# JackShDr/InfluentialRS

Measured on AMD Instinct MI355X. Metric: scored user-item pairs/sec (whole node), higher is better.
Workload: dtype f32; 1 GPU; c2: n_item=3415, d=128, L=200, H=4, layers=6, ffn=256; one greedy path-search step; users_per_gpu=4096, top_k=100, sweep=bf16 filter + exact f32 re-score, parallelism=single GPU

## Files before the change

influentialrs_amd/csrc/decoder.hip:

```cpp
#include "irs_internal.h"

typedef __attribute__((ext_vector_type(16))) float f32x16;

__global__ void __launch_bounds__(256) k_embed(const int64_t *__restrict__ seq, const float *__restrict__ E,
                                               const float *__restrict__ pe, float *__restrict__ x, int rows, int L,
                                               int d, float sqrtd, int64_t n_item) {
    int row = blockIdx.x * 4 + (threadIdx.x >> 6);
    int lane = threadIdx.x & 63;
    if (row >= rows) return;
    int64_t id = seq[row];
    if (id < 0) id = 0;
    if (id > n_item) id = n_item;
    int t = row % L;
    const float *e = E + id * (int64_t)d;
    const float *p = pe + (int64_t)t * d;
    float *o = x + (int64_t)row * d;
    for (int c = lane; c < d; c += 64) o[c] = __fadd_rn(__fmul_rn(e[c], sqrtd), p[c]);
}

__global__ void k_pif(const int64_t *__restrict__ user, const float *__restrict__ U, const float *__restrict__ w,
                      const float *__restrict__ b, float *__restrict__ r_u, int B, int ud, int64_t n_user) {
    int i = blockIdx.x * blockDim.x + threadIdx.x;
    if (i >= B) return;
    int64_t u = user[i];
    if (u < 0) u = 0;
    if (u >= n_user) u = n_user - 1;
    const float *e = U + u * (int64_t)ud;
    float acc = 0.f;
    for (int c = 0; c < ud; ++c) acc = __fmaf_rn(e[c], w[c], acc);
    r_u[i] = acc + b[0];
}

__global__ void k_fill(float *p, float v, int n) {
    int i = blockIdx.x * blockDim.x + threadIdx.x;
    if (i < n) p[i] = v;
}

__global__ void k_cross_const(const float *__restrict__ Wo, const float *__restrict__ b_in, const float *__restrict__ bo,
                              float *__restrict__ c, int d) {
    int i = blockIdx.x * blockDim.x + threadIdx.x;
    if (i >= d) return;
    const float *bv = b_in + 2 * d;
    float acc = 0.f;
    for (int j = 0; j < d; ++j) acc = __fmaf_rn(Wo[(int64_t)i * d + j], bv[j], acc);
    c[i] = acc + bo[i];
}

__device__ __forceinline__ bool plan_valid(const int64_t *__restrict__ sq, int t, int L, int p) {
    return t < L && (sq[t] != 0 || t == p);
}

__global__ void __launch_bounds__(256) k_plan_count(const int64_t *__restrict__ seq, const int32_t *__restrict__ pos, int B,
                                                    int L, int32_t *__restrict__ cnt, int32_t *__restrict__ tile_seq) {
    const int b = blockIdx.x * 4 + (threadIdx.x >> 6), lane = threadIdx.x & 63;
    if (b >= B) return;
    if (tile_seq && lane < 16) tile_seq[16 * b + lane] = -1;
    int p = pos[b];
    p = p < 0 ? 0 : (p >= L ? L - 1 : p);
    const int64_t *sq = seq + (int64_t)b * L;
    int n = 0;
    for (int t0 = 0; t0 < L; t0 += 64) n += __popcll(__ballot(plan_valid(sq, t0 + lane, L, p)));
    if (lane == 0) cnt[b] = n;
}

__global__ void __launch_bounds__(1024) k_plan_scan(const int32_t *__restrict__ cnt, int B, int32_t *__restrict__ off,
                                                    int32_t *__restrict__ m_dev) {
    __shared__ int s_scan[1024];
    __shared__ int s_base;
    const int tid = threadIdx.x;
    if (tid == 0) s_base = 0;
    __syncthreads();
    for (int b0 = 0; b0 < B; b0 += 1024) {
        const int b = b0 + tid;
        const int n = (b < B) ? cnt[b] : 0;
        s_scan[tid] = n;
        __syncthreads();
        for (int o = 1; o < 1024; o <<= 1) {
            int v = (tid >= o) ? s_scan[tid - o] : 0;
            __syncthreads();
            s_scan[tid] += v;
            __syncthreads();
        }
        const int base = s_base;
        if (b < B) off[b] = base + s_scan[tid] - n;
        __syncthreads();
        if (tid == 1023) s_base = base + s_scan[1023];
        __syncthreads();
    }
    if (tid == 0) m_dev[0] = s_base;
}

__global__ void __launch_bounds__(256) k_plan_fill(const int64_t *__restrict__ seq, const int32_t *__restrict__ pos, int B,
                                                   int L, const int32_t *__restrict__ off, int32_t *__restrict__ qrow,
                                                   int32_t *__restrict__ tok_row, int32_t *__restrict__ padq) {
    const int b = blockIdx.x * 4 + (threadIdx.x >> 6), lane = threadIdx.x & 63;
    if (b >= B) return;
    int p = pos[b];
    p = p < 0 ? 0 : (p >= L ? L - 1 : p);
    const int64_t *sq = seq + (int64_t)b * L;
    int o = off[b];
    for (int t0 = 0; t0 < L; t0 += 64) {
        const int t = t0 + lane;
        const bool v = plan_valid(sq, t, L, p);
        const unsigned long long m = __ballot(v);
        if (v) {
            const int idx = o + __popcll(m & ((1ull << lane) - 1ull));
            tok_row[idx] = b * L + t;
            if (t == p) {
                qrow[b] = idx;
                padq[b] = (sq[t] == 0) ? idx - off[b] : -1;
            }
        }
        o += __popcll(m);
    }
}

static int irs_cu_count() {
    static int n_cu = 0;
    if (n_cu == 0) {
        int dev = 0;
        if (hipGetDevice(&dev) != hipSuccess ||
            hipDeviceGetAttribute(&n_cu, hipDeviceAttributeMultiprocessorCount, dev) != hipSuccess || n_cu <= 0)
            n_cu = 256;
    }
    return n_cu;
}

#define SEQ_WG_TILES 8
#define SEQ_WG_BLOCKS 16
#define SEQ_AUTO_MIN_SEQS 384
#define SEQ_RMAX 48
#define SEQ_TAIL_BLOCKS 8
#ifndef SEQ_LAB_PLAN
#define SEQ_LAB_PLAN 0
#endif
__host__ __device__ __forceinline__ int seq_half_of_block(bool slot_odd, int nb, int blk) {
    const int mir = nb - 1 - blk;
    if (!slot_odd) {
        if ((nb & 1) && blk == mir) return nb - 1;
        return blk < mir ? 2 * blk : 2 * mir + 1;
    }
    if (nb & 1) {
        if (blk == mir) return 0;
        return blk < mir ? 1 + 2 * blk : 2 + 2 * mir;
    }
    if (blk == nb / 2 - 1) return 0;
    if (blk == nb / 2) return nb - 1;
    return blk < mir ? 1 + 2 * blk : 2 + 2 * mir;
}
#define SEQ_PLAN_PER_THREAD 8
__global__ void __launch_bounds__(1024) k_plan_seq(const int32_t *__restrict__ cnt, const int32_t *__restrict__ off,
                                                   const int32_t *__restrict__ qrow, int B, int32_t *__restrict__ tile_seq,
                                                   int32_t *__restrict__ tile_qb, int32_t *__restrict__ seq_row0,
                                                   int32_t *__restrict__ qrow_tile, int32_t *__restrict__ n_wg, int tiles_cap,
                                                   int n_cu) {
    constexpr int C = SEQ_WG_BLOCKS, PT = SEQ_PLAN_PER_THREAD, CT = SEQ_TAIL_BLOCKS;
    __shared__ int s_hist[C + 1], s_start[C + 2];
    __shared__ int p_n[C], p_s[C][SEQ_RMAX], p_l[C][SEQ_RMAX];
    __shared__ int c_cum[C + 1], c_q[C], c_exist, c_newbase, s_nwg;
    __shared__ int s_cap, s_tail0, c_norm, c_nnorm;
    __shared__ unsigned short s_order[1024 * PT], s_pt[1024 * PT];
    const int tid = threadIdx.x;
    if (tid <= C) s_hist[tid] = 0;
    if (tid < C) p_n[tid] = 0;
    if (tid == 0) s_nwg = 0, s_tail0 = -1;
    __syncthreads();
    int my_T[PT], my_rk[PT];
#pragma unroll
    for (int j = 0; j < PT; ++j) {
        const int b = tid + 1024 * j;
        my_T[j] = 0, my_rk[j] = 0;
        if (b < B) {
            int nb = (cnt[b] + 15) >> 4;
            nb = nb < 1 ? 1 : (nb > C ? C : nb);
            my_T[j] = nb;
            int pt = qrow[b] - off[b];
            s_pt[b] = (unsigned short)(pt < 0 ? 0 : (pt > 65535 ? 65535 : pt));
        }
    }
#pragma unroll
    for (int j = 0; j < PT; ++j)
        if (my_T[j]) my_rk[j] = atomicAdd(&s_hist[my_T[j]], 1);
    __syncthreads();
    if (tid == 0) {
        int run = 0;
        for (int T = C; T >= 1; --T) {
            s_start[T] = run;
            run += s_hist[T];
        }
        auto count = [&](const int cap, int &nwg, int &nbig, int &ntail) __attribute__((always_inline)) {
            int dc[C];
            nwg = 0, nbig = 0, ntail = 0;
#pragma unroll
            for (int f = 0; f < C; ++f) dc[f] = 0;
#pragma unroll
            for (int T = C; T >= 1; --T) {
                int left = s_hist[T];
                if (left > 0) {
#pragma unroll
                    for (int f = T; f < C; ++f) {
                        const int q = f / T, have = dc[f] * q, used = left < have ? left : have;
                        if (used > 0) {
                            const int fl = used / q, pa = used - fl * q;
                            left -= used;
                            dc[f] -= fl + (pa ? 1 : 0), dc[f - T * q] += fl;
#pragma unroll
                            for (int p = 1; p < q; ++p)
                                if (pa == p) dc[f - T * p] += 1;
                        }
                    }
                    const int q = C / T;
                    if (T <= CT) {
                        const int qt = T <= CT ? CT / T : 1, room = cap > nwg ? cap - nwg : 0;
                        if ((long long)room * q < left) {
                            const int tl = left - room * q, flt = tl / qt, pat = tl - flt * qt;
                            left = room * q;
                            dc[CT - T * qt] += flt, nwg += flt + (pat ? 1 : 0), ntail += flt + (pat ? 1 : 0);
#pragma unroll
                            for (int p = 1; p < qt; ++p)
                                if (pat == p) dc[CT - T * p] += 1;
                        }
                    }
                    const int fl = left / q, pa = left - fl * q;
                    dc[C - T * q] += fl, nwg += fl + (pa ? 1 : 0);
#pragma unroll
                    for (int p = 1; p < q; ++p)
                        if (pa == p) dc[C - T * p] += 1;
                }
                if (T == CT + 1) nbig = nwg;
            }
        };
        int nwg, nbig, ntail;
        count(0x7FFFFFFF, nwg, nbig, ntail);
        const int rounds = n_cu > 0 ? nwg / n_cu : 0, rem = nwg - rounds * n_cu;
        s_cap = 0x7FFFFFFF;
        if (SEQ_LAB_PLAN == 0 && n_cu > 0 && rem > 0 && 2 * rem <= n_cu && nbig <= rounds * n_cu) {
            int nwg2, nbig2;
            count(rounds * n_cu, nwg2, nbig2, ntail);
            if (ntail <= n_cu) s_cap = rounds * n_cu;
        }
        if (SEQ_LAB_PLAN == 1) s_cap = 0;
        if (SEQ_LAB_PLAN == 2) s_cap = 0x7FFFFFFF;
    }
    __syncthreads();
#pragma unroll
    for (int j = 0; j < PT; ++j)
        if (my_T[j]) s_order[s_start[my_T[j]] + my_rk[j]] = (unsigned short)(tid + 1024 * j);
    __syncthreads();
    auto pool_bins = [&](int f) {
        int n = 0;
        for (int r = 0; r < p_n[f]; ++r) n += p_l[f][r];
        return n;
    };
    auto append = [&](int f, int start, int len) {
        if (f < 1 || len < 1) return;
        if (p_n[f] > 0 && p_s[f][p_n[f] - 1] + p_l[f][p_n[f] - 1] == start) p_l[f][p_n[f] - 1] += len;
        else if (p_n[f] < SEQ_RMAX) p_s[f][p_n[f]] = start, p_l[f][p_n[f]] = len, ++p_n[f];
    };
    auto take_prefix = [&](int f, int m, int dest) {
        for (int r = 0; r < p_n[f] && m > 0; ++r) {
            const int t = m < p_l[f][r] ? m : p_l[f][r];
            append(dest, p_s[f][r], t);
            p_s[f][r] += t, p_l[f][r] -= t, m -= t;
        }
        int w = 0;
        for (int r = 0; r < p_n[f]; ++r)
            if (p_l[f][r] > 0) p_s[f][w] = p_s[f][r], p_l[f][w] = p_l[f][r], ++w;
        p_n[f] = w;
    };
    for (int T = C; T >= 1; --T) {
        const int n = s_hist[T], qnew = C / T;
        if (n == 0) continue;
        if (tid == 0) {
            int tot = 0;
            for (int f = T; f < C; ++f) {
                c_cum[f] = tot, c_q[f] = f / T;
                tot += pool_bins(f) * c_q[f];
            }
            c_cum[C] = tot;
            c_exist = n < tot ? n : tot;
            c_newbase = s_nwg;
            const int nnew = n - c_exist, room = s_cap > s_nwg ? s_cap - s_nwg : 0;
            const bool spill = T <= CT && nnew > 0 && (long long)room * qnew < nnew;
            c_norm = spill ? room * qnew : nnew;
            c_nnorm = (c_norm + qnew - 1) / qnew;
            const int ntail = spill ? (nnew - c_norm + CT / T - 1) / (CT / T) : 0;
            if (ntail > 0 && s_tail0 < 0) s_tail0 = c_newbase + c_nnorm;
            s_nwg += c_nnorm + ntail;
        }
        __syncthreads();
        const int exist = c_exist, base = s_start[T];
        for (int i = tid; i < n; i += 1024) {
            const int b = s_order[base + i];
            int w, slot;
            if (i < exist) {
                int f = T;
                while (f < C - 1 && i >= c_cum[f + 1]) ++f;
                const int s_ = i - c_cum[f];
                int bl = s_ / c_q[f];
                const int k = s_ % c_q[f];
                int r = 0;
                while (r < p_n[f] - 1 && bl >= p_l[f][r]) bl -= p_l[f][r], ++r;
                w = p_s[f][r] + bl;
                slot = (C - f) + k * T;
            } else if (i - exist < c_norm) {
                const int j_ = i - exist;
                w = c_newbase + j_ / qnew;
                slot = (j_ % qnew) * T;
            } else {
                const int j_ = i - exist - c_norm, qt = CT / T;
                w = c_newbase + c_nnorm + j_ / qt;
                slot = (C - CT) + (j_ % qt) * T;
            }
            if (w * SEQ_WG_TILES >= tiles_cap) continue;
            const int h0 = 2 * SEQ_WG_TILES * w + slot;
            for (int blk = 0; blk < T; ++blk) {
                const int h = h0 + seq_half_of_block(slot & 1, T, blk);
                tile_seq[h] = b, tile_qb[h] = blk;
            }
            seq_row0[b] = 16 * slot;
            const int pt = s_pt[b];
            int pb = pt >> 4;
            pb = pb < 0 ? 0 : (pb >= T ? T - 1 : pb);
            qrow_tile[b] = 16 * (h0 + seq_half_of_block(slot & 1, T, pb)) + (pt & 15);
        }
        __syncthreads();
        if (tid == 0) {
            int left = exist;
            for (int f = T; f < C && left > 0; ++f) {
                const int q = c_q[f], cap = pool_bins(f) * q;
                const int used = left < cap ? left : cap;
                left -= used;
                const int full = used / q, part = used % q;
                take_prefix(f, full, f - T * q);
                if (part) take_prefix(f, 1, f - T * part);
            }
            const int nnew = c_norm, fullnew = nnew / qnew, partnew = nnew % qnew;
            append(C - T * qnew, c_newbase, fullnew);
            if (partnew) append(C - T * partnew, c_newbase + fullnew, 1);
            if (n - exist > c_norm) {
                const int ntl = n - exist - c_norm, qt = CT / T, fullt = ntl / qt, partt = ntl % qt;
                append(CT - T * qt, c_newbase + c_nnorm, fullt);
                if (partt) append(CT - T * partt, c_newbase + c_nnorm + fullt, 1);
            }
        }
        __syncthreads();
    }
    if (tid == 0) n_wg[0] = s_nwg, n_wg[1] = s_tail0 < 0 ? s_nwg : s_tail0;
}

__global__ void __launch_bounds__(1024) k_plan_small(const int64_t *__restrict__ seq, const int32_t *__restrict__ pos, int B, int L,
                                                     int32_t *__restrict__ cnt, int32_t *__restrict__ off,
                                                     int32_t *__restrict__ qrow, int32_t *__restrict__ tok_row,
                                                     int32_t *__restrict__ padq, int32_t *__restrict__ m_dev,
                                                     const int64_t *__restrict__ user, const float *__restrict__ U,
                                                     const float *__restrict__ uw, const float *__restrict__ ub,
                                                     float *__restrict__ r_u, int ud, int64_t n_user,
                                                     int32_t *__restrict__ step_pair) {
    __shared__ int s_cnt[64], s_off[64];
    const int tid = threadIdx.x, wave = tid >> 6, lane = tid & 63;
    for (int b = wave; b < B; b += 16) {
        int p = pos[b];
        p = p < 0 ? 0 : (p >= L ? L - 1 : p);
        const int64_t *sq = seq + (int64_t)b * L;
        int n = 0;
        for (int t0 = 0; t0 < L; t0 += 64) n += __popcll(__ballot(plan_valid(sq, t0 + lane, L, p)));
        if (lane == 0) s_cnt[b] = n;
    }
    if (tid < B) {
        float acc = 0.f;
        if (U) {
            int64_t u = user[tid];
            if (u < 0) u = 0;
            if (u >= n_user) u = n_user - 1;
            const float *e = U + u * (int64_t)ud;
            for (int c = 0; c < ud; ++c) acc = __fmaf_rn(e[c], uw[c], acc);
            acc += ub[0];
        }
        r_u[tid] = acc;
    }
    __syncthreads();
    if (tid == 0) {
        int run = 0;
        for (int b = 0; b < B; ++b) {
            s_off[b] = run;
            run += s_cnt[b];
        }
        m_dev[0] = run;
        if (step_pair) step_pair[0] = step_pair[1];
    }
    __syncthreads();
    for (int b = wave; b < B; b += 16) {
        int p = pos[b];
        p = p < 0 ? 0 : (p >= L ? L - 1 : p);
        const int64_t *sq = seq + (int64_t)b * L;
        int o = s_off[b];
        if (lane == 0) {
            cnt[b] = s_cnt[b];
            off[b] = o;
        }
        const int o0 = o;
        for (int t0 = 0; t0 < L; t0 += 64) {
            const int t = t0 + lane;
            const bool v = plan_valid(sq, t, L, p);
            const unsigned long long m = __ballot(v);
            if (v) {
                const int idx = o + __popcll(m & ((1ull << lane) - 1ull));
                tok_row[idx] = b * L + t;
                if (t == p) {
                    qrow[b] = idx;
                    padq[b] = (sq[t] == 0) ? idx - o0 : -1;
                }
            }
            o += __popcll(m);
        }
    }
}

__global__ void __launch_bounds__(256) k_embed_packed(const int64_t *__restrict__ seq, const float *__restrict__ E,
                                                      const float *__restrict__ pe, float *__restrict__ x,
                                                      const int32_t *__restrict__ tok_row, const int32_t *__restrict__ m_dev,
                                                      int L, int d, float sqrtd, int64_t n_item) {
    const int row = blockIdx.x * 4 + (threadIdx.x >> 6);
    const int lane = threadIdx.x & 63;
    if (row >= m_dev[0]) return;
    const int orig = tok_row[row];
    int64_t id = seq[orig];
    if (id < 0) id = 0;
    if (id > n_item) id = n_item;
    const float *e = E + id * (int64_t)d;
    const float *p = pe + (int64_t)(orig % L) * d;
// ... 5358 lines not shown
    case DecFam::FRAG_FUSED:
        return frag_layer(c, l);
    case DecFam::SMALL16:
    case DecFam::WIDE:
    case DecFam::ANY: {
        SmallBlockArgs sb = small_args(ctx, r.layer, l, ctx->act_ao, x, nullptr, y, qkv_buf(c, l + 1), c.rows, c.m_dev,
                                       l + 1 < ctx->dims.n_layers);
        if (r.att_fused) {
            sb.QKVin = qkv_buf(c, l), sb.r_u = ctx->act_ru, sb.seq_last = c.seq + (ctx->dims.max_len - 1), sb.cnt = c.cnt;
            sb.padq = ctx->seq_padq, sb.mask_mode = ctx->dims.mask_mode;
        }
        launch_small(ctx, r.layer, sb, r.att_fused, c.rows > SMALL_MT2_ROWS, c.s);
        c.x = y;
        c.y = x;
        return IRS_OK;
    }
    default:
        return gemm_rest(ctx, r.layer == DecFam::GEMM_LN, l, ctx->act_ao, x, r.layer == DecFam::GEMM_LN ? y : x, y, x, c.rows, c.m_dev,
                         c.s);
    }
}

static int last_layer(const DecodeCall &c, int l, const int32_t *pos, float *xrows) {
    irs_ctx *ctx = c.ctx;
    const DecodeRoute &r = c.r;
    const int L = ctx->dims.max_len, d = ctx->dims.d, H = ctx->dims.n_heads, B = c.B;
    const irs_layer_w &w = ctx->layer[l];
    const int32_t *qrow = c.qrow;
    const hipStream_t s = c.s;
    int rc;
    float *xf = ctx->act_xf, *h_r = ctx->act_h;
    float *ao_r = ctx->act_ao, *x_r = ao_r + (size_t)B * d, *y_r = ao_r + (size_t)2 * B * d, *z_r = ao_r + (size_t)3 * B * d;
    const float *q_r = nullptr;
    const int nt = d > 128 ? d / 32 : 4;
    if (r.seq) {
#if SEQ_LAST_ABSORB
        float *um = ctx->act_h, *cq = um + (size_t)B * 4 * d;
        hipLaunchKernelGGL(k_absorb_qu, dim3((B + ABS_SQ - 1) / ABS_SQ), dim3(256), 0, s, xf, ctx->qrow_tile, w.sa_in_w, w.sa_in_b, x_r, um,
                           cq, B);
        hipLaunchKernelGGL(k_absorb_attn, dim3(B), dim3(256), 0, s, xf, um, cq, c.seq, ctx->act_ru, L, ctx->dims.mask_mode, c.off, c.cnt,
                           qrow, ctx->seq_padq, ctx->seq_row0, ctx->qrow_tile);
        hipLaunchKernelGGL(k_absorb_out, dim3((B + ABS_SO - 1) / ABS_SO), dim3(256), 0, s, um, w.sa_in_w, w.sa_in_b, ao_r, B);
#else
        hipLaunchKernelGGL(k_gather_rows_frag, dim3(B), dim3(64), 0, s, xf, ctx->qrow_tile, x_r, d, nt);
        hipLaunchKernelGGL(k_gather_rows_frag, dim3(B), dim3(64), 0, s, ctx->act_yf, ctx->qrow_tile, ao_r, d, nt);
#endif
    } else if (r.kv_only) {
        hipLaunchKernelGGL(k_gather_rows_frag, dim3(B), dim3(64), 0, s, xf, qrow, x_r, d, nt);
        LinArgs q{};
        q.X = x_r, q.W = w.sa_in_w, q.bias = w.sa_in_b, q.Y = h_r, q.M = B, q.N = d, q.K = d;
        if ((rc = launch_linear(ctx, q, s))) return rc;
        q_r = h_r;
    }
    irs_prof_begin(ctx, IRS_PROF_ATTN, s);
    if (r.seq) {
    } else if (d / H == 32 && L <= 256 && d % 4 == 0 && (((uintptr_t)ctx->act_qkv | (uintptr_t)q_r) & 15) == 0)
        hipLaunchKernelGGL(k_attn_row32, dim3(H, B), dim3(256), 0, s, ctx->act_qkv, c.seq, ctx->act_ru, ao_r, L, d,
                           ctx->dims.mask_mode, c.off, c.cnt, qrow, q_r, ctx->seq_padq);
    else
        hipLaunchKernelGGL(k_attn_row, dim3(H, B), dim3(64), 0, s, ctx->act_qkv, c.seq, ctx->act_ru, pos, ao_r, L, d, d / H,
                           ctx->dims.mask_mode, c.off, c.cnt, c.tok, qrow, q_r);
    irs_prof_end(ctx, IRS_PROF_ATTN, s, 4.0 * B * (double)L * d, 4.0 * 3.0 * B * (double)L * d);
    const bool small = r.tail == DecFam::SMALL16 || r.tail == DecFam::WIDE || r.tail == DecFam::ANY;
    const bool idx_res = small && !r.frag;
    if (r.frag && !r.kv_only) hipLaunchKernelGGL(k_gather_rows_frag, dim3(B), dim3(64), 0, s, xf, qrow, x_r, d, nt);
    else if (!r.frag && !idx_res) hipLaunchKernelGGL(k_gather_rows_idx, dim3(B), dim3(64), 0, s, c.x, qrow, x_r, d);
    if (small) {
        const SmallBlockArgs sb = small_args(ctx, r.tail, l, ao_r, idx_res ? c.x : x_r, idx_res ? qrow : nullptr, xrows, nullptr, B,
                                             nullptr, false);
        launch_small(ctx, r.tail, sb, false, B > 2048, s);
    } else if ((rc = gemm_rest(ctx, r.tail == DecFam::GEMM_LN, l, ao_r, x_r, y_r, z_r, xrows, B, nullptr, s))) {
        return rc;
    }
    IRS_CHECK_HIP(ctx, hipGetLastError());
    return IRS_OK;
}

int irs_launch_decode(irs_ctx *ctx, const int64_t *seq, const int64_t *user, int B, float *x_out, const int32_t *pos,
                      float *xrows, float *r_u_out, hipStream_t s) {
    const int L = ctx->dims.max_len, d = ctx->dims.d, nl = ctx->dims.n_layers;
    const DecodeRoute r = decode_route(ctx, B, x_out == nullptr && pos && xrows && L >= 4);
    int rc;
    if (ctx->step_pair && !r.small_plan) IRS_FAIL(ctx, IRS_E_STATE, "merged path step needs the single-workgroup plan kernel");
    if (!r.small_plan && (rc = irs_launch_pif(ctx, user, B, ctx->act_ru, s)) != IRS_OK) return rc;
    ctx->seq_last = r.seq;
    const int32_t packed[IRS_ROUTE_FIELDS] = {r.rows_only, r.small_plan, (int32_t)r.plan, (int32_t)r.embed, (int32_t)r.layer,
                                              (int32_t)r.tail, r.frag, r.seq, r.kv_planes, r.att_fused, r.kv_only, r.x6, r.npl, r.nt};
    for (int i = 0; i < IRS_ROUTE_FIELDS; ++i) ctx->route_last[i] = packed[i];
    ctx->route_n = IRS_ROUTE_FIELDS;
    DecodeCall c{ctx, r, seq, B, B * L, ctx->act_x, ctx->act_y, s};
    if (r.rows_only) c.off = ctx->seq_off, c.cnt = ctx->seq_cnt, c.tok = ctx->tok_row, c.qrow = ctx->seq_qrow, c.m_dev = ctx->m_dev;
    if (r.plan == DecPlan::SMALL) {
        hipLaunchKernelGGL(k_plan_small, dim3(1), dim3(1024), 0, s, seq, pos, B, L, ctx->seq_cnt, ctx->seq_off, ctx->seq_qrow,
                           ctx->tok_row, ctx->seq_padq, ctx->m_dev, user, pif_table(ctx), ctx->um_w, ctx->um_b, ctx->act_ru,
                           ctx->dims.u_dim, ctx->dims.n_user, ctx->step_pair);
    } else if (r.plan == DecPlan::MULTI) {
        hipLaunchKernelGGL(k_plan_count, dim3((B + 3) / 4), dim3(256), 0, s, seq, pos, B, L, ctx->seq_cnt, ctx->tile_seq);
        hipLaunchKernelGGL(k_plan_scan, dim3(1), dim3(1024), 0, s, ctx->seq_cnt, B, ctx->seq_off, ctx->m_dev);
        hipLaunchKernelGGL(k_plan_fill, dim3((B + 3) / 4), dim3(256), 0, s, seq, pos, B, L, ctx->seq_off, ctx->seq_qrow, ctx->tok_row,
                           ctx->seq_padq);
    }
    const int n_cu = r.seq ? irs_cu_count() : 0;
    if (r.seq)
        hipLaunchKernelGGL(k_plan_seq, dim3(1), dim3(1024), 0, s, ctx->seq_cnt, ctx->seq_off, ctx->seq_qrow, B, ctx->tile_seq,
                           ctx->tile_idx, ctx->seq_row0, ctx->qrow_tile, ctx->n_wg_dev, B * SEQ_WG_TILES, n_cu);
    launch_embed(c, pos, user);
    IRS_CHECK_HIP(ctx, hipGetLastError());
    if (r_u_out) IRS_CHECK_HIP(ctx, hipMemcpyAsync(r_u_out, ctx->act_ru, sizeof(float) * B, hipMemcpyDeviceToDevice, s));
    const bool embed_qkv = r.embed == DecEmbed::SEQ || r.embed == DecEmbed::FRAG_QKV || r.embed == DecEmbed::SMALL16_QKV ||
                           r.embed == DecEmbed::ANY_QKV;
    const int l0 = r.seq ? nl - 1 : 0;
    for (int l = l0; l < nl; ++l) {
        const irs_layer_w &w = ctx->layer[l];
        if (!(l == l0 ? embed_qkv : fam_writes_qkv(r.layer))) {
            LinArgs q{};
            q.X = c.x, q.Xf = r.frag ? ctx->act_xf : nullptr, q.W = w.sa_in_w, q.bias = w.sa_in_b, q.Y = ctx->act_qkv;
            q.M = c.rows, q.N = 3 * d, q.K = d, q.m_dev = c.m_dev;
            if ((rc = launch_linear(ctx, q, s))) return rc;
        }
        if (r.rows_only && l + 1 == nl) return last_layer(c, l, pos, xrows);
        if ((rc = decode_layer(c, l))) return rc;
        IRS_CHECK_HIP(ctx, hipGetLastError());
    }
    if (x_out) IRS_CHECK_HIP(ctx, hipMemcpyAsync(x_out, c.x, sizeof(float) * (size_t)c.rows * d, hipMemcpyDeviceToDevice, s));
    if (pos && xrows) {
        hipLaunchKernelGGL(k_gather_rows, dim3(B), dim3(64), 0, s, c.x, pos, xrows, B, L, d);
        IRS_CHECK_HIP(ctx, hipGetLastError());
    }
    return IRS_OK;
}
```

influentialrs_amd/csrc/irs_internal.h:

```cpp
#pragma once

#include <hip/hip_runtime.h>
#include <stdint.h>
#include <stdio.h>
#include <string.h>

#include "../../include/irs_hip.h"

#if !defined(IRS_LAB) && (defined(X6_DUMP) || defined(X6_STAMP) || defined(X6_NO_SPLIT) || defined(X6_STAGGER) ||            \
                          defined(X6_NO_MFMA) || defined(X6_NO_READS) || defined(X6_NO_DMA) || defined(X6_NO_BARRIER) ||       \
                          defined(X6_NW) || defined(ATTN_STAMP) || defined(ATTNP_STAMP) ||               \
                          defined(IRS_SMALL_TIMING) || defined(IRS_DIRECT_TIMING) || defined(SWEEP_LAB) || defined(X6D_STAMP) ||              \
                          defined(X6_NO_QKV_STORE) || defined(X6_NSLOT2) || defined(X6_RESID_LATE) || defined(X6_RING4) ||      \
                          defined(X6_SPLIT_ACC4) || defined(SEQ_EXP))
#error "a lab switch (X6_* / ATTN* / IRS_*_TIMING) is defined without IRS_LAB: the product library must be built without them"
#endif

#include <atomic>
#include <functional>
#define IRS_MAX_DEVICES 32
static inline int irs_cur_dev() {
    int d = 0;
    if (hipGetDevice(&d) != hipSuccess || d < 0 || d >= IRS_MAX_DEVICES) d = 0;
    return d;
}
#define IRS_ONCE_PER_DEVICE(body_)                                                                                        \
    do {                                                                                                                  \
        static std::atomic<unsigned> once_mask_{0};                                                                       \
        const unsigned once_bit_ = 1u << irs_cur_dev();                                                                   \
        if (!(once_mask_.load(std::memory_order_acquire) & once_bit_)) {                                                  \
            body_;                                                                                                        \
            once_mask_.fetch_or(once_bit_, std::memory_order_release);                                                    \
        }                                                                                                                 \
    } while (0)

#define IRS_MAX_LAYERS 16
#define IRS_CAND_BUCKETS 64
#define IRS_CAND_SLOTS 64
#define IRS_CAND_CAP (IRS_CAND_BUCKETS * IRS_CAND_SLOTS)
#define IRS_REFINE_CAP 1024
#define IRS_MAX_GROUPS 2048
#define IRS_MAX_PATH 64
#define IRS_MAX_EXCL 4096
#define IRS_LSE_SLOTS_RING 4096
#define IRS_COOP_FALLBACK_MIN_ITEMS 262144
#define IRS_EXH_SCRATCH_KEYS (64 * 32768)

struct irs_layer_w {
    const float *sa_in_w, *sa_in_b, *sa_out_w, *sa_out_b;
    const float *ca_in_w, *ca_in_b, *ca_out_w, *ca_out_b;
    const float *l1_w, *l1_b, *l2_w, *l2_b;
    const float *n1_w, *n1_b, *n2_w, *n2_b, *n3_w, *n3_b;
};

struct irs_prof_ev {
    hipEvent_t a, b;
};

enum { IRS_STEP_GREEDY = 1, IRS_STEP_BEAM, IRS_STEP_SHARDED_BEAM, IRS_STEP_SHARDED_BEAM_SPLIT };
struct irs_step_key {
    int32_t kind, B, W, P, k, sweep, sample, sample_k;
    uint64_t seed;
    const void *comm, *seq, *user, *hep, *paths, *status;
};
static_assert(sizeof(irs_step_key) == 8 * sizeof(int32_t) + 7 * 8, "irs_step_key is compared with memcmp: no padding");
struct irs_step_graph {
    hipGraphExec_t exec;
    irs_step_key key;
};

struct irs_excl {
    const int64_t *rows;
    const int32_t *cnt;
    const int32_t *map;
    const float *paths;
    const int32_t *step_ptr;
    int stride, div;
    int path_ld, path_by_user;
    int step_arg, on;
};

struct irs_beam_state {
    int64_t *seq;
    int32_t *hep;
    double *cum;
    float *paths;
    int32_t *fin;
};
struct irs_beam_side {
    int64_t *user;
    int32_t *done;
    int32_t *map;
};
struct irs_beam_cand {
    const float *val;
    const int64_t *ids0;
    const float *lse_max, *lse_sum;
// ... 484 lines not shown
```

Measured before the change: 2.323 billion pairs/s.

## Restructure multi-sequence plan pipeline: fuse PIF, drop scan kernel, parallelize seq placement

```diff
diff --git a/influentialrs_amd/csrc/decoder.hip b/influentialrs_amd/csrc/decoder.hip
--- a/influentialrs_amd/csrc/decoder.hip
+++ b/influentialrs_amd/csrc/decoder.hip
@@ -51,7 +51,10 @@
 }
 
 __global__ void __launch_bounds__(256) k_plan_count(const int64_t *__restrict__ seq, const int32_t *__restrict__ pos, int B,
-                                                    int L, int32_t *__restrict__ cnt, int32_t *__restrict__ tile_seq) {
+                                                    int L, int32_t *__restrict__ cnt, int32_t *__restrict__ tile_seq,
+                                                    const int64_t *__restrict__ user, const float *__restrict__ U, const float *__restrict__ w,
+                                                    const float *__restrict__ bias, float *__restrict__ r_u, int ud,
+                                                    int64_t n_user) {
     const int b = blockIdx.x * 4 + (threadIdx.x >> 6), lane = threadIdx.x & 63;
     if (b >= B) return;
     if (tile_seq && lane < 16) tile_seq[16 * b + lane] = -1;
@@ -60,45 +63,252 @@
     const int64_t *sq = seq + (int64_t)b * L;
     int n = 0;
     for (int t0 = 0; t0 < L; t0 += 64) n += __popcll(__ballot(plan_valid(sq, t0 + lane, L, p)));
-    if (lane == 0) cnt[b] = n;
-}
-
-__global__ void __launch_bounds__(1024) k_plan_scan(const int32_t *__restrict__ cnt, int B, int32_t *__restrict__ off,
-                                                    int32_t *__restrict__ m_dev) {
-    __shared__ int s_scan[1024];
-    __shared__ int s_base;
+    float acc = 0.f;
+    if (U) {
+        int64_t u = user[b];
+        if (u < 0) u = 0;
+        if (u >= n_user) u = n_user - 1;
+        const float *e = U + u * (int64_t)ud;
+        for (int c0 = 0; c0 < ud; c0 += 64) {
+            const bool in = c0 + lane < ud;
+            const float ev = in ? e[c0 + lane] : 0.f, wv = in ? w[c0 + lane] : 0.f;
+            const int nc = ud - c0 < 64 ? ud - c0 : 64;
+            for (int c = 0; c < nc; ++c) acc = __fmaf_rn(__shfl(ev, c), __shfl(wv, c), acc);
+        }
+        acc = acc + bias[0];
+    }
+    if (lane == 0) {
+        cnt[b] = n;
+        r_u[b] = acc;
+    }
+}
+
+static int irs_cu_count() {
+    static int n_cu = 0;
+    if (n_cu == 0) {
+        int dev = 0;
+        if (hipGetDevice(&dev) != hipSuccess ||
+            hipDeviceGetAttribute(&n_cu, hipDeviceAttributeMultiprocessorCount, dev) != hipSuccess || n_cu <= 0)
+            n_cu = 256;
+    }
+    return n_cu;
+}
+
+#define SEQ_WG_TILES 8
+#define SEQ_WG_BLOCKS 16
+#define SEQ_AUTO_MIN_SEQS 384
+#define SEQ_TAIL_BLOCKS 8
+#ifndef SEQ_LAB_PLAN
+#define SEQ_LAB_PLAN 0
+#endif
+__host__ __device__ __forceinline__ int seq_half_of_block(bool slot_odd, int nb, int blk) {
+    const int mir = nb - 1 - blk;
+    if (!slot_odd) {
+        if ((nb & 1) && blk == mir) return nb - 1;
+        return blk < mir ? 2 * blk : 2 * mir + 1;
+    }
+    if (nb & 1) {
+        if (blk == mir) return 0;
+        return blk < mir ? 1 + 2 * blk : 2 + 2 * mir;
+    }
+    if (blk == nb / 2 - 1) return 0;
+    if (blk == nb / 2) return nb - 1;
+    return blk < mir ? 1 + 2 * blk : 2 + 2 * mir;
+}
+#define SEQ_PLAN_PER_THREAD 8
+#ifdef PLAN_STAMP
+__device__ unsigned long long g_plan_t[32];
+extern "C" void *irs_lab_plan_stamps() {
+    void *p = nullptr;
+    return hipGetSymbolAddress(&p, HIP_SYMBOL(g_plan_t)) == hipSuccess ? p : nullptr;
+}
+#define PSTAMP(i) do { if (threadIdx.x == 0) g_plan_t[i] = __builtin_amdgcn_s_memtime(); } while (0)
+#else
+#define PSTAMP(i)
+#endif
+__global__ void __launch_bounds__(1024) k_plan_seq(const int32_t *__restrict__ cnt, int B, int32_t *__restrict__ place,
+                                                   int32_t *__restrict__ n_wg, int n_cu) {
+    constexpr int C = SEQ_WG_BLOCKS, PT = SEQ_PLAN_PER_THREAD, CT = SEQ_TAIL_BLOCKS;
+    __shared__ int s_hist[C + 1], s_start[C + 2];
+    __shared__ int c_cum[2][C + 1][C], c_exist[2][C + 1], c_newbase[2][C + 1], c_norm[2][C + 1], c_nnorm[2][C + 1], c_ntail[2][C + 1];
+    __shared__ int s_rank[C + 1][C];
+    __shared__ int s_sel, s_nwg;
+    __shared__ unsigned short s_first[1024 * PT];
     const int tid = threadIdx.x;
-    if (tid == 0) s_base = 0;
+    PSTAMP(0);
+    if (tid <= C) s_hist[tid] = 0;
+    if (tid < (C + 1) * C) (&s_rank[0][0])[tid] = 0;
     __syncthreads();
-    for (int b0 = 0; b0 < B; b0 += 1024) {
-        const int b = b0 + tid;
-        const int n = (b < B) ? cnt[b] : 0;
-        s_scan[tid] = n;
-        __syncthreads();
-        for (int o = 1; o < 1024; o <<= 1) {
-            int v = (tid >= o) ? s_scan[tid - o] : 0;
-            __syncthreads();
-            s_scan[tid] += v;
-            __syncthreads();
-        }
-        const int base = s_base;
-        if (b < B) off[b] = base + s_scan[tid] - n;
-        __syncthreads();
-        if (tid == 1023) s_base = base + s_scan[1023];
-        __syncthreads();
-    }
-    if (tid == 0) m_dev[0] = s_base;
+    int my_T[PT], my_rk[PT];
+#pragma unroll
+    for (int j = 0; j < PT; ++j) {
+        const int b = tid + 1024 * j;
+        my_T[j] = 0, my_rk[j] = 0;
+        if (b < B) {
+            int nb = (cnt[b] + 15) >> 4;
+            nb = nb < 1 ? 1 : (nb > C ? C : nb);
+            my_T[j] = nb;
+        }
+    }
+#pragma unroll
+    for (int j = 0; j < PT; ++j)
+        if (my_T[j]) my_rk[j] = atomicAdd(&s_hist[my_T[j]], 1);
+    __syncthreads();
+    if (tid >= 1 && tid <= C) {
+        int run = 0;
+        for (int U = C; U > tid; --U) run += s_hist[U];
+        s_start[tid] = run;
+    }
+    __syncthreads();
+    PSTAMP(1);
+    if (tid == 0) {
+        auto count = [&](const int cap, const int set, int &nwg, int &nbig, int &ntail, int &tail0) __attribute__((always_inline)) {
+            int dc[C];
+            nwg = 0, nbig = 0, ntail = 0, tail0 = -1;
+#pragma unroll
+            for (int f = 0; f < C; ++f) dc[f] = 0;
+#pragma unroll
+            for (int T = C; T >= 1; --T) {
+                const int n = s_hist[T];
+                int left = n;
+                if (left > 0) {
+                    int tot = 0;
+#pragma unroll
+                    for (int f = T; f < C; ++f) {
+                        const int q = f / T, have = dc[f] * q, used = left < have ? left : have;
+                        c_cum[set][T][f] = tot;
+                        tot += have;
+                        if (used > 0) {
+                            const int fl = used / q, pa = used - fl * q;
+                            left -= used;
+                            dc[f] -= fl + (pa ? 1 : 0), dc[f - T * q] += fl;
+#pragma unroll
+                            for (int p = 1; p < q; ++p)
+                                if (pa == p) dc[f - T * p] += 1;
+                        }
+                    }
+                    c_exist[set][T] = n - left, c_newbase[set][T] = nwg;
+                    const int q = C / T, base0 = nwg;
+                    int ntl = 0;
+                    if (T <= CT) {
+                        const int qt = T <= CT ? CT / T : 1, room = cap > nwg ? cap - nwg : 0;
+                        if ((long long)room * q < left) {
+                            const int tl = left - room * q, flt = tl / qt, pat = tl - flt * qt;
+                            left = room * q;
+                            ntl = flt + (pat ? 1 : 0);
+                            dc[CT - T * qt] += flt, nwg += ntl, ntail += ntl;
+#pragma unroll
+                            for (int p = 1; p < qt; ++p)
+                                if (pat == p) dc[CT - T * p] += 1;
+                        }
+                    }
+                    const int fl = left / q, pa = left - fl * q;
+                    dc[C - T * q] += fl, nwg += fl + (pa ? 1 : 0);
+#pragma unroll
+                    for (int p = 1; p < q; ++p)
+                        if (pa == p) dc[C - T * p] += 1;
+                    c_norm[set][T] = left, c_nnorm[set][T] = fl + (pa ? 1 : 0), c_ntail[set][T] = ntl;
+                    if (ntl > 0 && tail0 < 0) tail0 = base0 + fl + (pa ? 1 : 0);
+                }
+                if (T == CT + 1) nbig = nwg;
+            }
+        };
+        int nwg, nbig, ntail, tail0, sel = 0;
+        count(0x7FFFFFFF, 0, nwg, nbig, ntail, tail0);
+        const int rounds = n_cu > 0 ? nwg / n_cu : 0, rem = nwg - rounds * n_cu;
+        if (SEQ_LAB_PLAN == 1 || (SEQ_LAB_PLAN == 0 && n_cu > 0 && rem > 0 && 2 * rem <= n_cu && nbig <= rounds * n_cu)) {
+            int nwg2, nbig2, ntail2, tail02;
+            count(SEQ_LAB_PLAN == 1 ? 0 : rounds * n_cu, 1, nwg2, nbig2, ntail2, tail02);
+            if (SEQ_LAB_PLAN == 1 || ntail2 <= n_cu) sel = 1, nwg = nwg2, tail0 = tail02;
+        }
+        s_sel = sel, s_nwg = nwg;
+        n_wg[0] = nwg, n_wg[1] = tail0 < 0 ? nwg : tail0;
+    }
+    __syncthreads();
+    PSTAMP(2);
+    const int sel = s_sel, nwg_all = s_nwg;
+    int wf[PT];
+#pragma unroll
+    for (int k = 0; k < PT; ++k) wf[k] = 0;
+    for (int T = C; T >= 1; --T) {
+        const int n = s_hist[T];
+        if (n == 0) continue;
+        const int exist = c_exist[sel][T], newbase = c_newbase[sel][T], nnorm = c_nnorm[sel][T], ntl = c_ntail[sel][T],
+                  base = s_start[T];
+#pragma unroll
+        for (int k = 0; k < PT; ++k) {
+            const int w = tid + 1024 * k;
+            if (1024 * k >= nwg_all) break;
+            if (w < newbase) {
+                const int f = wf[k];
+                if (f >= T && exist > 0) {
+                    const int q = f / T, i0 = c_cum[sel][T][f] + q * atomicAdd(&s_rank[T][f], 1);
+                    if (i0 < exist) {
+                        s_first[base + i0] = (unsigned short)w;
+                        wf[k] = f - T * (exist - i0 < q ? exist - i0 : q);
+                    }
+                }
+            } else if (w < newbase + nnorm) {
+                const int qnew = C / T, j_ = w - newbase, norm = c_norm[sel][T];
+                wf[k] = C - T * (norm - j_ * qnew < qnew ? norm - j_ * qnew : qnew);
+            } else if (w < newbase + nnorm + ntl) {
+                const int qt = CT / T, j_ = w - newbase - nnorm, left = n - exist - c_norm[sel][T];
+                wf[k] = CT - T * (left - j_ * qt < qt ? left - j_ * qt : qt);
+            }
+        }
+    }
+    __syncthreads();
+    PSTAMP(3);
+#pragma unroll
+    for (int j = 0; j < PT; ++j) {
+        const int T = my_T[j], i = my_rk[j];
+        if (T == 0) continue;
+        const int exist = c_exist[sel][T], norm = c_norm[sel][T], qnew = C / T;
+        int w, slot;
+        if (i < exist) {
+            int f = T;
+            while (f < C - 1 && i >= c_cum[sel][T][f + 1]) ++f;
+            const int s_ = i - c_cum[sel][T][f], q = f / T, r = s_ / q;
+            w = s_first[s_start[T] + c_cum[sel][T][f] + r * q];
+            slot = (C - f) + (s_ - r * q) * T;
+        } else if (i - exist < norm) {
+            const int j_ = i - exist;
+            w = c_newbase[sel][T] + j_ / qnew;
+            slot = (j_ % qnew) * T;
+        } else {
+            const int j_ = i - exist - norm, qt = T <= CT ? CT / T : 1;
+            w = c_newbase[sel][T] + c_nnorm[sel][T] + j_ / qt;
+            slot = (C - CT) + (j_ % qt) * T;
+        }
+        place[tid + 1024 * j] = 16 * w + slot;
+    }
+#ifdef PLAN_STAMP
+    if ((tid & 63) == 0) g_plan_t[16 + (tid >> 6)] = __builtin_amdgcn_s_memtime();
+#endif
 }
 
 __global__ void __launch_bounds__(256) k_plan_fill(const int64_t *__restrict__ seq, const int32_t *__restrict__ pos, int B,
-                                                   int L, const int32_t *__restrict__ off, int32_t *__restrict__ qrow,
-                                                   int32_t *__restrict__ tok_row, int32_t *__restrict__ padq) {
-    const int b = blockIdx.x * 4 + (threadIdx.x >> 6), lane = threadIdx.x & 63;
+                                                   int L, const int32_t *__restrict__ cnt, int32_t *__restrict__ off,
+                                                   int32_t *__restrict__ qrow, int32_t *__restrict__ tok_row,
+                                                   int32_t *__restrict__ padq, int32_t *__restrict__ m_dev,
+                                                   int32_t *__restrict__ tile_seq, int32_t *__restrict__ tile_qb,
+                                                   int32_t *__restrict__ seq_row0, int32_t *__restrict__ qrow_tile, int tiles_cap) {
+    __shared__ int s_part[4];
+    const int wave = threadIdx.x >> 6, b = blockIdx.x * 4 + wave, lane = threadIdx.x & 63;
+    int base = 0;
+    for (int i = threadIdx.x; i < 4 * (int)blockIdx.x; i += 256) base += cnt[i];
+    for (int o = 32; o >= 1; o >>= 1) base += __shfl_xor(base, o);
+    if (lane == 0) s_part[wave] = base;
+    __syncthreads();
     if (b >= B) return;
+    int o = s_part[0] + s_part[1] + s_part[2] + s_part[3];
+    for (int i = 4 * blockIdx.x; i < b; ++i) o += cnt[i];
+    const int ob = o;
     int p = pos[b];
     p = p < 0 ? 0 : (p >= L ? L - 1 : p);
     const int64_t *sq = seq + (int64_t)b * L;
-    int o = off[b];
+    if (lane == 0) off[b] = ob;
+    int below = 0;
     for (int t0 = 0; t0 < L; t0 += 64) {
         const int t = t0 + lane;
         const bool v = plan_valid(sq, t, L, p);
@@ -108,245 +318,30 @@
             tok_row[idx] = b * L + t;
             if (t == p) {
                 qrow[b] = idx;
-                padq[b] = (sq[t] == 0) ? idx - off[b] : -1;
-            }
-        }
+                padq[b] = (sq[t] == 0) ? idx - ob : -1;
+            }
+        }
+        const int nlow = p - t0;
+        below += __popcll(m & (nlow >= 64 ? ~0ull : (nlow <= 0 ? 0ull : (1ull << nlow) - 1ull)));
         o += __popcll(m);
     }
-}
-
-static int irs_cu_count() {
-    static int n_cu = 0;
-    if (n_cu == 0) {
-        int dev = 0;
-        if (hipGetDevice(&dev) != hipSuccess ||
-            hipDeviceGetAttribute(&n_cu, hipDeviceAttributeMultiprocessorCount, dev) != hipSuccess || n_cu <= 0)
-            n_cu = 256;
-    }
-    return n_cu;
-}
-
-#define SEQ_WG_TILES 8
-#define SEQ_WG_BLOCKS 16
-#define SEQ_AUTO_MIN_SEQS 384
-#define SEQ_RMAX 48
-#define SEQ_TAIL_BLOCKS 8
-#ifndef SEQ_LAB_PLAN
-#define SEQ_LAB_PLAN 0
-#endif
-__host__ __device__ __forceinline__ int seq_half_of_block(bool slot_odd, int nb, int blk) {
-    const int mir = nb - 1 - blk;
-    if (!slot_odd) {
-        if ((nb & 1) && blk == mir) return nb - 1;
-        return blk < mir ? 2 * blk : 2 * mir + 1;
-    }
-    if (nb & 1) {
-        if (blk == mir) return 0;
-        return blk < mir ? 1 + 2 * blk : 2 + 2 * mir;
-    }
-    if (blk == nb / 2 - 1) return 0;
-    if (blk == nb / 2) return nb - 1;
-    return blk < mir ? 1 + 2 * blk : 2 + 2 * mir;
-}
-#define SEQ_PLAN_PER_THREAD 8
-__global__ void __launch_bounds__(1024) k_plan_seq(const int32_t *__restrict__ cnt, const int32_t *__restrict__ off,
-                                                   const int32_t *__restrict__ qrow, int B, int32_t *__restrict__ tile_seq,
-                                                   int32_t *__restrict__ tile_qb, int32_t *__restrict__ seq_row0,
-                                                   int32_t *__restrict__ qrow_tile, int32_t *__restrict__ n_wg, int tiles_cap,
-                                                   int n_cu) {
-    constexpr int C = SEQ_WG_BLOCKS, PT = SEQ_PLAN_PER_THREAD, CT = SEQ_TAIL_BLOCKS;
-    __shared__ int s_hist[C + 1], s_start[C + 2];
-    __shared__ int p_n[C], p_s[C][SEQ_RMAX], p_l[C][SEQ_RMAX];
-    __shared__ int c_cum[C + 1], c_q[C], c_exist, c_newbase, s_nwg;
-    __shared__ int s_cap, s_tail0, c_norm, c_nnorm;
-    __shared__ unsigned short s_order[1024 * PT], s_pt[1024 * PT];
-    const int tid = threadIdx.x;
-    if (tid <= C) s_hist[tid] = 0;
-    if (tid < C) p_n[tid] = 0;
-    if (tid == 0) s_nwg = 0, s_tail0 = -1;
-    __syncthreads();
-    int my_T[PT], my_rk[PT];
-#pragma unroll
-    for (int j = 0; j < PT; ++j) {
-        const int b = tid + 1024 * j;
-        my_T[j] = 0, my_rk[j] = 0;
-        if (b < B) {
-            int nb = (cnt[b] + 15) >> 4;
-            nb = nb < 1 ? 1 : (nb > C ? C : nb);
-            my_T[j] = nb;
-            int pt = qrow[b] - off[b];
-            s_pt[b] = (unsigned short)(pt < 0 ? 0 : (pt > 65535 ? 65535 : pt));
-        }
-    }
-#pragma unroll
-    for (int j = 0; j < PT; ++j)
-        if (my_T[j]) my_rk[j] = atomicAdd(&s_hist[my_T[j]], 1);
-    __syncthreads();
-    if (tid == 0) {
-        int run = 0;
-        for (int T = C; T >= 1; --T) {
-            s_start[T] = run;
-            run += s_hist[T];
-        }
-        auto count = [&](const int cap, int &nwg, int &nbig, int &ntail) __attribute__((always_inline)) {
-            int dc[C];
-            nwg = 0, nbig = 0, ntail = 0;
-#pragma unroll
-            for (int f = 0; f < C; ++f) dc[f] = 0;
-#pragma unroll
-            for (int T = C; T >= 1; --T) {
-                int left = s_hist[T];
-                if (left > 0) {
-#pragma unroll
-                    for (int f = T; f < C; ++f) {
-                        const int q = f / T, have = dc[f] * q, used = left < have ? left : have;
-                        if (used > 0) {
-                            const int fl = used / q, pa = used - fl * q;
-                            left -= used;
-                            dc[f] -= fl + (pa ? 1 : 0), dc[f - T * q] += fl;
-#pragma unroll
-                            for (int p = 1; p < q; ++p)
-                                if (pa == p) dc[f - T * p] += 1;
-                        }
-                    }
-                    const int q = C / T;
-                    if (T <= CT) {
-                        const int qt = T <= CT ? CT / T : 1, room = cap > nwg ? cap - nwg : 0;
-                        if ((long long)room * q < left) {
-                            const int tl = left - room * q, flt = tl / qt, pat = tl - flt * qt;
-                            left = room * q;
-                            dc[CT - T * qt] += flt, nwg += flt + (pat ? 1 : 0), ntail += flt + (pat ? 1 : 0);
-#pragma unroll
-                            for (int p = 1; p < qt; ++p)
-                                if (pat == p) dc[CT - T * p] += 1;
-                        }
-                    }
-                    const int fl = left / q, pa = left - fl * q;
-                    dc[C - T * q] += fl, nwg += fl + (pa ? 1 : 0);
-#pragma unroll
-                    for (int p = 1; p < q; ++p)
-                        if (pa == p) dc[C - T * p] += 1;
-                }
-                if (T == CT + 1) nbig = nwg;
-            }
-        };
-        int nwg, nbig, ntail;
-        count(0x7FFFFFFF, nwg, nbig, ntail);
-        const int rounds = n_cu > 0 ? nwg / n_cu : 0, rem = nwg - rounds * n_cu;
-        s_cap = 0x7FFFFFFF;
-        if (SEQ_LAB_PLAN == 0 && n_cu > 0 && rem > 0 && 2 * rem <= n_cu && nbig <= rounds * n_cu) {
-            int nwg2, nbig2;
-            count(rounds * n_cu, nwg2, nbig2, ntail);
-            if (ntail <= n_cu) s_cap = rounds * n_cu;
-        }
-        if (SEQ_LAB_PLAN == 1) s_cap = 0;
-        if (SEQ_LAB_PLAN == 2) s_cap = 0x7FFFFFFF;
-    }
-    __syncthreads();
-#pragma unroll
-    for (int j = 0; j < PT; ++j)
-        if (my_T[j]) s_order[s_start[my_T[j]] + my_rk[j]] = (unsigned short)(tid + 1024 * j);
-    __syncthreads();
-    auto pool_bins = [&](int f) {
-        int n = 0;
-        for (int r = 0; r < p_n[f]; ++r) n += p_l[f][r];
-        return n;
-    };
-    auto append = [&](int f, int start, int len) {
-        if (f < 1 || len < 1) return;
-        if (p_n[f] > 0 && p_s[f][p_n[f] - 1] + p_l[f][p_n[f] - 1] == start) p_l[f][p_n[f] - 1] += len;
-        else if (p_n[f] < SEQ_RMAX) p_s[f][p_n[f]] = start, p_l[f][p_n[f]] = len, ++p_n[f];
-    };
-    auto take_prefix = [&](int f, int m, int dest) {
-        for (int r = 0; r < p_n[f] && m > 0; ++r) {
-            const int t = m < p_l[f][r] ? m : p_l[f][r];
-            append(dest, p_s[f][r], t);
-            p_s[f][r] += t, p_l[f][r] -= t, m -= t;
-        }
-        int w = 0;
-        for (int r = 0; r < p_n[f]; ++r)
-            if (p_l[f][r] > 0) p_s[f][w] = p_s[f][r], p_l[f][w] = p_l[f][r], ++w;
-        p_n[f] = w;
-    };
-    for (int T = C; T >= 1; --T) {
-        const int n = s_hist[T], qnew = C / T;
-        if (n == 0) continue;
-        if (tid == 0) {
-            int tot = 0;
-            for (int f = T; f < C; ++f) {
-                c_cum[f] = tot, c_q[f] = f / T;
-                tot += pool_bins(f) * c_q[f];
-            }
-            c_cum[C] = tot;
-            c_exist = n < tot ? n : tot;
-            c_newbase = s_nwg;
-            const int nnew = n - c_exist, room = s_cap > s_nwg ? s_cap - s_nwg : 0;
-            const bool spill = T <= CT && nnew > 0 && (long long)room * qnew < nnew;
-            c_norm = spill ? room * qnew : nnew;
-            c_nnorm = (c_norm + qnew - 1) / qnew;
-            const int ntail = spill ? (nnew - c_norm + CT / T - 1) / (CT / T) : 0;
-            if (ntail > 0 && s_tail0 < 0) s_tail0 = c_newbase + c_nnorm;
-            s_nwg += c_nnorm + ntail;
-        }
-        __syncthreads();
-        const int exist = c_exist, base = s_start[T];
-        for (int i = tid; i < n; i += 1024) {
-            const int b = s_order[base + i];
-            int w, slot;
-            if (i < exist) {
-                int f = T;
-                while (f < C - 1 && i >= c_cum[f + 1]) ++f;
-                const int s_ = i - c_cum[f];
-                int bl = s_ / c_q[f];
-                const int k = s_ % c_q[f];
-                int r = 0;
-                while (r < p_n[f] - 1 && bl >= p_l[f][r]) bl -= p_l[f][r], ++r;
-                w = p_s[f][r] + bl;
-                slot = (C - f) + k * T;
-            } else if (i - exist < c_norm) {
-                const int j_ = i - exist;
-                w = c_newbase + j_ / qnew;
-                slot = (j_ % qnew) * T;
-            } else {
-                const int j_ = i - exist - c_norm, qt = CT / T;
-                w = c_newbase + c_nnorm + j_ / qt;
-                slot = (C - CT) + (j_ % qt) * T;
-            }
-            if (w * SEQ_WG_TILES >= tiles_cap) continue;
-            const int h0 = 2 * SEQ_WG_TILES * w + slot;
-            for (int blk = 0; blk < T; ++blk) {
-                const int h = h0 + seq_half_of_block(slot & 1, T, blk);
-                tile_seq[h] = b, tile_qb[h] = blk;
-            }
-            seq_row0[b] = 16 * slot;
-            const int pt = s_pt[b];
-            int pb = pt >> 4;
-            pb = pb < 0 ? 0 : (pb >= T ? T - 1 : pb);
-            qrow_tile[b] = 16 * (h0 + seq_half_of_block(slot & 1, T, pb)) + (pt & 15);
-        }
-        __syncthreads();
-        if (tid == 0) {
-            int left = exist;
-            for (int f = T; f < C && left > 0; ++f) {
-                const int q = c_q[f], cap = pool_bins(f) * q;
-                const int used = left < cap ? left : cap;
-                left -= used;
-                const int full = used / q, part = used % q;
-                take_prefix(f, full, f - T * q);
-                if (part) take_prefix(f, 1, f - T * part);
-            }
-            const int nnew = c_norm, fullnew = nnew / qnew, partnew = nnew % qnew;
-            append(C - T * qnew, c_newbase, fullnew);
-            if (partnew) append(C - T * partnew, c_newbase + fullnew, 1);
-            if (n - exist > c_norm) {
-                const int ntl = n - exist - c_norm, qt = CT / T, fullt = ntl / qt, partt = ntl % qt;
-                append(CT - T * qt, c_newbase + c_nnorm, fullt);
-                if (partt) append(CT - T * partt, c_newbase + c_nnorm + fullt, 1);
-            }
-        }
-        __syncthreads();
-    }
-    if (tid == 0) n_wg[0] = s_nwg, n_wg[1] = s_tail0 < 0 ? s_nwg : s_tail0;
+    if (b == B - 1 && lane == 0) m_dev[0] = o;
+    if (!tile_seq) return;
+    int T = (o - ob + 15) >> 4;
+    T = T < 1 ? 1 : (T > SEQ_WG_BLOCKS ? SEQ_WG_BLOCKS : T);
+    const int pl = seq_row0[b], w = pl >> 4, slot = pl & 15;
+    if (w < 0 || w * SEQ_WG_TILES >= tiles_cap || slot + T > SEQ_WG_BLOCKS) return;
+    const int h0 = 2 * SEQ_WG_TILES * w + slot;
+    if (lane < T) {
+        const int h = h0 + seq_half_of_block(slot & 1, T, lane);
+        tile_seq[h] = b, tile_qb[h] = lane;
+    }
+    if (lane == 0) {
+        seq_row0[b] = 16 * slot;
+        int pb = below >> 4;
+        pb = pb >= T ? T - 1 : pb;
+        qrow_tile[b] = 16 * (h0 + seq_half_of_block(slot & 1, T, pb)) + (below & 15);
+    }
 }
 
 __global__ void __launch_bounds__(1024) k_plan_small(const int64_t *__restrict__ seq, const int32_t *__restrict__ pos, int B, int L,
@@ -5871,7 +5866,7 @@
     const DecodeRoute r = decode_route(ctx, B, x_out == nullptr && pos && xrows && L >= 4);
     int rc;
     if (ctx->step_pair && !r.small_plan) IRS_FAIL(ctx, IRS_E_STATE, "merged path step needs the single-workgroup plan kernel");
-    if (!r.small_plan && (rc = irs_launch_pif(ctx, user, B, ctx->act_ru, s)) != IRS_OK) return rc;
+    if (r.plan == DecPlan::NONE && (rc = irs_launch_pif(ctx, user, B, ctx->act_ru, s)) != IRS_OK) return rc;
     ctx->seq_last = r.seq;
     const int32_t packed[IRS_ROUTE_FIELDS] = {r.rows_only, r.small_plan, (int32_t)r.plan, (int32_t)r.embed, (int32_t)r.layer,
                                               (int32_t)r.tail, r.frag, r.seq, r.kv_planes, r.att_fused, r.kv_only, r.x6, r.npl, r.nt};
@@ -5884,15 +5879,14 @@
                            ctx->tok_row, ctx->seq_padq, ctx->m_dev, user, pif_table(ctx), ctx->um_w, ctx->um_b, ctx->act_ru,
                            ctx->dims.u_dim, ctx->dims.n_user, ctx->step_pair);
     } else if (r.plan == DecPlan::MULTI) {
-        hipLaunchKernelGGL(k_plan_count, dim3((B + 3) / 4), dim3(256), 0, s, seq, pos, B, L, ctx->seq_cnt, ctx->tile_seq);
-        hipLaunchKernelGGL(k_plan_scan, dim3(1), dim3(1024), 0, s, ctx->seq_cnt, B, ctx->seq_off, ctx->m_dev);
-        hipLaunchKernelGGL(k_plan_fill, dim3((B + 3) / 4), dim3(256), 0, s, seq, pos, B, L, ctx->seq_off, ctx->seq_qrow, ctx->tok_row,
-                           ctx->seq_padq);
-    }
-    const int n_cu = r.seq ? irs_cu_count() : 0;
-    if (r.seq)
-        hipLaunchKernelGGL(k_plan_seq, dim3(1), dim3(1024), 0, s, ctx->seq_cnt, ctx->seq_off, ctx->seq_qrow, B, ctx->tile_seq,
-                           ctx->tile_idx, ctx->seq_row0, ctx->qrow_tile, ctx->n_wg_dev, B * SEQ_WG_TILES, n_cu);
+        hipLaunchKernelGGL(k_plan_count, dim3((B + 3) / 4), dim3(256), 0, s, seq, pos, B, L, ctx->seq_cnt, ctx->tile_seq, user,
+                           pif_table(ctx), ctx->um_w, ctx->um_b, ctx->act_ru, ctx->dims.u_dim, ctx->dims.n_user);
+        if (r.seq)
+            hipLaunchKernelGGL(k_plan_seq, dim3(1), dim3(1024), 0, s, ctx->seq_cnt, B, ctx->seq_row0, ctx->n_wg_dev, irs_cu_count());
+        hipLaunchKernelGGL(k_plan_fill, dim3((B + 3) / 4), dim3(256), 0, s, seq, pos, B, L, ctx->seq_cnt, ctx->seq_off, ctx->seq_qrow,
+                           ctx->tok_row, ctx->seq_padq, ctx->m_dev, r.seq ? ctx->tile_seq : nullptr, ctx->tile_idx, ctx->seq_row0,
+                           ctx->qrow_tile, B * SEQ_WG_TILES);
+    }
     launch_embed(c, pos, user);
     IRS_CHECK_HIP(ctx, hipGetLastError());
     if (r_u_out) IRS_CHECK_HIP(ctx, hipMemcpyAsync(r_u_out, ctx->act_ru, sizeof(float) * B, hipMemcpyDeviceToDevice, s));
diff --git a/influentialrs_amd/csrc/irs_internal.h b/influentialrs_amd/csrc/irs_internal.h
--- a/influentialrs_amd/csrc/irs_internal.h
+++ b/influentialrs_amd/csrc/irs_internal.h
@@ -12,7 +12,7 @@
                           defined(X6_NW) || defined(ATTN_STAMP) || defined(ATTNP_STAMP) ||               \
                           defined(IRS_SMALL_TIMING) || defined(IRS_DIRECT_TIMING) || defined(SWEEP_LAB) || defined(X6D_STAMP) ||              \
                           defined(X6_NO_QKV_STORE) || defined(X6_NSLOT2) || defined(X6_RESID_LATE) || defined(X6_RING4) ||      \
-                          defined(X6_SPLIT_ACC4) || defined(SEQ_EXP))
+                          defined(X6_SPLIT_ACC4) || defined(SEQ_EXP) || defined(PLAN_STAMP))
 #error "a lab switch (X6_* / ATTN* / IRS_*_TIMING) is defined without IRS_LAB: the product library must be built without them"
 #endif
 
```

After: 2.360 billion pairs/s (median of 6 runs). 1.02x the previous value.
